# 77even/Fast-nnUNet

Measured on AMD Instinct MI355X. Metric: 3d_fullres patches/sec (distilled r=2 student, sliding window, one 512^3 CT; volume resident in HBM at step start; step ends with: fp16 logits resident in HBM), higher is better.
Workload: dtype f16; 1 GPU; bone_turbo_r2: PlainConvUNet student r=2, features [16, 32, 64, 128, 160, 160], 1 input channel, patch 160x96x96, 61 classes, 512^3 volume, tile_step_size 0.5, Gaussian on, mirroring off, 600 patches/volume; patches_per_forward=32, folds=1, accumulators=fp16, step_output=fp16 logits [heads, X, Y, Z] in HBM (predict_sliding_window_return_logits), gpu_max_hw_queues=4, parallelism=single GPU

## Files before the change

fast-nnunet_amd/csrc/conv3d_row.hip:

```cpp
#include "fnn_device.h"
#include "conv_common.h"
#include <cstdlib>

namespace {

struct RowCur { int n, d, h0, g; };

template <int NBLK, int CH, bool TCONV>
__global__ __launch_bounds__(256, CH == 1 ? (NBLK <= 8 ? 3 : 2) : (NBLK <= 8 ? 2 : 1)) void conv_row_kernel(const ThinParams tp, const int total_units,
                                                                         const int strips, const int SH) {
    extern __shared__ __attribute__((aligned(16))) char smem[];
    const ConvParams &p = tp.c;
    constexpr int W = 16 * NBLK, PB = (W + 2) * 32, RINGB = 12 * PB;
    constexpr int PF = NBLK / 2;
    constexpr int NPL = TCONV ? 1 : CH;
    constexpr int TB = TCONV ? (NBLK + 3) / 4 : 1;
    const int tid = threadIdx.x, lane = tid & 63, r = lane & 15, q = lane >> 4, hl = lane >> 5, kh = q & 1;
    const int wave = __builtin_amdgcn_readfirstlane(tid >> 6);
    const int H = p.Hi, D = p.Di, G = SH >> 2;
    double *sRed = (double *)(smem + CH * RINGB);

    int u_begin, u_end;
    {
        const int nwg = gridDim.x, bid = blockIdx.x;
        const int g = fnn_xcd_tile(nwg, bid);
        u_begin = (int)((long long)total_units * g / nwg);
        u_end = (int)((long long)total_units * (g + 1) / nwg);
    }
    if (u_begin >= u_end) return;
    const int n_groups = (u_end - u_begin) * (G + 1);
    auto advance = [&](RowCur &c) {
        if (++c.g > G) {
            c.g = 0; c.h0 += SH;
            if (c.h0 >= H) { c.h0 = 0; if (++c.d >= D) { c.d = 0; ++c.n; } }
        }
    };

    if (tid < CH * 12 * 4) {
        const int row = tid >> 2, which = (tid >> 1) & 1, half = tid & 1;
        *(f16x8 *)(smem + row * PB + (which ? (W + 1) * 32 : 0) + half * 16) = (f16x8){0, 0, 0, 0, 0, 0, 0, 0};
    }
    for (int i = tid; i < 4 * 16 * 2; i += 256) sRed[i] = 0.0;
    const int cg = tid & 1;
    int e_row[PF], e_goff[PF], e_lds[PF];
#pragma unroll
    for (int u = 0; u < PF; ++u) {
        const int e = tid + 256 * u, i = e / (2 * W), c = e - i * (2 * W), col = (c >> 1) + 1;
        e_row[u] = __builtin_amdgcn_readfirstlane(i);
        e_goff[u] = c * 16;
        e_lds[u] = col * 32 + ((cg ^ ((col >> 2) & 1)) * 16);
    }
    int lanec[5];
#pragma unroll
    for (int ks = 0; ks < 5; ++ks) {
        const int t = 2 * ks + hl < 9 ? 2 * ks + hl : 8;
        const int col = r + t % 3;
        lanec[ks] = col * 32 + ((kh ^ ((col >> 2) & 1)) * 16);
    }
    f16x8 wf[CH][5];
#pragma unroll
    for (int ch = 0; ch < CH; ++ch)
#pragma unroll
        for (int ks = 0; ks < 5; ++ks) wf[ch][ks] = *(const f16x8 *)(p.wpk + ((size_t)(ch * 5 + ks) * 64 + lane) * 8);
    const float4 bv = *(const float4 *)(p.bias + q * 4);
    f16x8 fwf[TCONV ? 4 : 1];
    f32x4 fb = {0.f, 0.f, 0.f, 0.f};
    int up_lds[2] = {0, 0};
    if (TCONV) {
#pragma unroll
        for (int cls = 0; cls < 4; ++cls) fwf[cls] = *(const f16x8 *)(tp.fw + ((size_t)cls * 64 + lane) * 8);
        const float4 t = *(const float4 *)(tp.fbias + q * 4);
        fb = (f32x4){t.x, t.y, t.z, t.w};
#pragma unroll
        for (int jw = 0; jw < 2; ++jw) {
            const int col = 2 * r + jw + 1;
            up_lds[jw] = col * 32 + (((q >> 1) ^ ((col >> 2) & 1)) * 16) + (q & 1) * 8;
        }
    }
    const size_t plane_rows = (size_t)H;
    const int Hl = tp.Hl, Wl = tp.Wl;

    f16x8 xr[NPL][PF];
    f16x8 xl[TB];
    f16x8 sc_h[NPL], sh_h[NPL];
    f16 slope_h[NPL];
    float lsc[8], lsh[8];
#ifndef FNN_NORM_FP32
    f16x8 lsc_h = {0, 0, 0, 0, 0, 0, 0, 0}, lsh_h = lsc_h;
#endif
    int n_ss = -1;
    auto load_ss = [&](int n) {
#pragma unroll
        for (int pc = 0; pc < NPL; ++pc) {
            const SrcDesc &S = p.src[TCONV ? 1 : pc];
            const float *qs, *qh;
            fnn_ss_rows(S.ss, 16, n, 0, p.ident_ss, qs, qh);
#pragma unroll
            for (int j = 0; j < 8; ++j) {
                sc_h[pc][j] = (f16)(cg ? qs[8 + j] : qs[j]);
                sh_h[pc][j] = (f16)(cg ? qh[8 + j] : qh[j]);
            }
            slope_h[pc] = (f16)S.slope;
        }
        if (TCONV) {
            const SrcDesc &S = tp.low;
            const float *qs, *qh;
            fnn_ss_rows(S.ss, 32, n, 0, p.ident_ss, qs, qh);
#pragma unroll
            for (int j = 0; j < 8; ++j) {
                lsc[j] = q == 0 ? qs[j] : q == 1 ? qs[8 + j] : q == 2 ? qs[16 + j] : qs[24 + j];
                lsh[j] = q == 0 ? qh[j] : q == 1 ? qh[8 + j] : q == 2 ? qh[16 + j] : qh[24 + j];
            }
#ifndef FNN_NORM_FP32
#pragma unroll
            for (int j = 0; j < 8; ++j) { lsc_h[j] = (f16)lsc[j]; lsh_h[j] = (f16)lsh[j]; }
#endif
        }
    };
    auto issue = [&](const RowCur &c) {
        const int rbase = c.h0 - 1 + 4 * c.g;
#pragma unroll
        for (int pc = 0; pc < NPL; ++pc) {
            const SrcDesc &S = p.src[TCONV ? 1 : pc];
#pragma unroll
            for (int u = 0; u < PF; ++u) {
                int row = rbase + e_row[u];
                row = row < 0 ? 0 : (row >= H ? H - 1 : row);
                const char *base = (const char *)(S.ptr + (((size_t)c.n * D + c.d) * plane_rows + row) * (W * 16));
                xr[pc][u] = *(const f16x8 *)(base + (unsigned)e_goff[u]);
            }
        }
        if (TCONV) {
            const int lbase = (c.h0 >> 1) - 1 + 2 * c.g;
#pragma unroll
            for (int t = 0; t < TB; ++t) {
                int bb = wave + 4 * t;
                bb = bb < NBLK ? bb : wave;
                const int lr = bb / (NBLK / 2), bl = bb - lr * (NBLK / 2);
                int lrow = lbase + lr;
                lrow = lrow < 0 ? 0 : (lrow >= Hl ? Hl - 1 : lrow);
                const char *base = (const char *)(tp.low.ptr + (size_t)c.n * tp.Dl * Hl * Wl * 32 + (q >> 1) * FNN_CS(tp.low) +
                                                  (((size_t)c.d * Hl + lrow) * Wl) * FNN_VS(tp.low));
                xl[t] = *(const f16x8 *)(base + (unsigned)((16 * bl + r) * (FNN_VS(tp.low) * 2) + (q & 1) * 16));
            }
        }
    };
    auto commit = [&](const RowCur &c, int slot) {
        if (c.n != n_ss) { load_ss(c.n); n_ss = c.n; }
        const int rbase = c.h0 - 1 + 4 * c.g;
#pragma unroll
        for (int pc = 0; pc < NPL; ++pc) {
            char *ring = smem + (TCONV ? 1 : pc) * RINGB;
#pragma unroll
            for (int u = 0; u < PF; ++u) {
                const int row = rbase + e_row[u];
                f16x8 o = xr[pc][u] * sc_h[pc] + sh_h[pc];
                o = __builtin_elementwise_max(o, o * slope_h[pc]);
                if (row < 0 || row >= H) o = (f16x8){0, 0, 0, 0, 0, 0, 0, 0};
                *(f16x8 *)(ring + (slot * 4 + e_row[u]) * PB + e_lds[u]) = o;
            }
        }
        if (TCONV) {
            const int lbase = (c.h0 >> 1) - 1 + 2 * c.g;
            const f16 lslope = (f16)tp.low.slope;
#pragma unroll
            for (int t = 0; t < TB; ++t) {
                const int bb = wave + 4 * t;
                if (bb < NBLK) {
                    const int lr = bb / (NBLK / 2), bl = bb - lr * (NBLK / 2);
                    const int lrow = lbase + lr;
                    const bool ok = lrow >= 0 && lrow < Hl;
#ifdef FNN_NORM_FP32
                    f16x8 o = fnn_norm8(xl[t], lsc, lsh);
#else
                    f16x8 o = xl[t] * lsc_h + lsh_h;
#endif
                    o = __builtin_elementwise_max(o, o * lslope);
                    char *dst = smem + (slot * 4 + 2 * lr) * PB + bl * 1024;
                    f32x4 dd[4];
#pragma unroll
                    for (int cls = 0; cls < 4; ++cls)
                        dd[cls] = __builtin_amdgcn_mfma_f32_16x16x32_f16(fwf[cls], o, (f32x4){0.f, 0.f, 0.f, 0.f}, 0, 0, 0);
                    __builtin_amdgcn_sched_barrier(0);
#pragma unroll
                    for (int cls = 0; cls < 4; ++cls) {
                        f16x4 h;
                        h[0] = (f16)(dd[cls][0] + fb[0]); h[1] = (f16)(dd[cls][1] + fb[1]); h[2] = (f16)(dd[cls][2] + fb[2]); h[3] = (f16)(dd[cls][3] + fb[3]);
                        if (!ok) h = (f16x4){0, 0, 0, 0};
                        *(f16x4 *)(dst + (cls >> 1) * PB + up_lds[cls & 1]) = h;
                    }
                }
            }
        }
    };

    double dsum[4][2];
#pragma unroll
    for (int j = 0; j < 4; ++j) { dsum[j][0] = 0.0; dsum[j][1] = 0.0; }
    auto flush_stats = [&](int n) {
        if (!p.stats_out) return;
#pragma unroll
        for (int j = 0; j < 4; ++j) {
            const double a = row16_sum_f64(dsum[j][0]), b = row16_sum_f64(dsum[j][1]);
            if (r == 0) { double *slot = sRed + (wave * 16 + q * 4 + j) * 2; slot[0] = a; slot[1] = b; }
            dsum[j][0] = 0.0; dsum[j][1] = 0.0;
        }
        __syncthreads();
        if (tid < 32) {
            const int c = tid >> 1, which = tid & 1;
            double v = 0;
#pragma unroll
            for (int w = 0; w < 4; ++w) { v += sRed[(w * 16 + c) * 2 + which]; sRed[(w * 16 + c) * 2 + which] = 0.0; }
            unsafeAtomicAdd(p.stats_out + (((size_t)n * FNN_STAT_REPL + (blockIdx.x & (FNN_STAT_REPL - 1))) * p.Cout + c) * 2 + which, v);
        }
        __syncthreads();
    };

    const unsigned out_lane = (unsigned)((r + 16 * (q & 1)) * 32 + (q >> 1) * 16);
    const f16x2 ones = {(f16)1.f, (f16)1.f};
    auto step = [&](const RowCur &c, int slot) {
        const int slot1 = slot == 2 ? 0 : slot + 1;
        f32x4 acc[NBLK];
#pragma unroll
        for (int b = 0; b < NBLK; ++b) acc[b] = (f32x4){0.f, 0.f, 0.f, 0.f};
#pragma unroll
        for (int ch = 0; ch < CH; ++ch) {
            const int sh0 = (TCONV && ch == 0) ? 1 : 0;
            int ro[3];
#pragma unroll
            for (int tr = 0; tr < 3; ++tr) {
                const int wi = wave + tr + sh0;
                ro[tr] = (wi < 4 ? slot * 4 + wi : slot1 * 4 + wi - 4) * PB;
            }
            const char *ring = smem + ch * RINGB;
#pragma unroll
            for (int ks = 0; ks < 5; ++ks) {
                const int vo = lanec[ks] + (ks == 1 ? (hl ? ro[1] : ro[0]) : ro[ks == 0 ? 0 : ks == 2 ? 1 : 2]);
                constexpr int BG = NBLK <= 8 ? NBLK : NBLK / 2;
#pragma unroll
                for (int b0 = 0; b0 < NBLK; b0 += BG) {
                    f16x8 xf[BG];
#pragma unroll
                    for (int b = 0; b < BG; ++b) xf[b] = *(const f16x8 *)(ring + vo + (b0 + b) * 512);
#pragma unroll
                    for (int b = 0; b < BG; ++b) acc[b0 + b] = __builtin_amdgcn_mfma_f32_16x16x32_f16(wf[ch][ks], xf[b], acc[b0 + b], 0, 0, 0);
                }
            }
        }
        const int orow = c.h0 + 4 * c.g + wave;
        char *obase = (char *)(p.out + (((size_t)c.n * D + c.d) * plane_rows + orow) * (W * 16));
        float t1[4] = {0.f, 0.f, 0.f, 0.f}, t2[4] = {0.f, 0.f, 0.f, 0.f};
#pragma unroll
        for (int b = 0; b < NBLK; b += 2) {
            f16x4 o[2];
#pragma unroll
            for (int h = 0; h < 2; ++h) {
                o[h][0] = (f16)(acc[b + h][0] + bv.x);
                o[h][1] = (f16)(acc[b + h][1] + bv.y);
                o[h][2] = (f16)(acc[b + h][2] + bv.z);
                o[h][3] = (f16)(acc[b + h][3] + bv.w);
            }
            *(fnn_u32x4r *)(obase + out_lane + b * 512) = pair_to_b128(o[0], o[1]);
#pragma unroll
            for (int j = 0; j < 4; ++j) {
                const f16x2 pr = {o[0][j], o[1][j]};
                t1[j] = __builtin_amdgcn_fdot2(pr, ones, t1[j], false);
                t2[j] = __builtin_amdgcn_fdot2(pr, pr, t2[j], false);
            }
        }
        if (p.stats_out) {
#pragma unroll
            for (int j = 0; j < 4; ++j) { dsum[j][0] += (double)t1[j]; dsum[j][1] += (double)t2[j]; }
        }
    };

    RowCur cc;
    {
        const int u = u_begin, strip = u % strips, pd = u / strips;
        cc.h0 = strip * SH; cc.d = pd % D; cc.n = pd / D; cc.g = 0;
    }
    RowCur cw = cc, ci = cc;
    int gw = 0, gl = 0;
    __syncthreads();
    issue(ci);
    commit(cw, 0);
    if (gl < n_groups - 1) { advance(ci); ++gl; }
    if (gw < n_groups - 1) { advance(cw); ++gw; }
    issue(ci);
    commit(cw, 1);
    if (gl < n_groups - 1) { advance(ci); ++gl; }
    if (gw < n_groups - 1) { advance(cw); ++gw; }
    issue(ci);
    __syncthreads();
    int slot = 0;
    for (int gi = 0; gi < n_groups; ++gi) {
        if (cc.g < G) step(cc, slot);
        commit(cw, slot == 0 ? 2 : slot - 1);
        if (gl < n_groups - 1) { advance(ci); ++gl; }
        if (gw < n_groups - 1) { advance(cw); ++gw; }
        issue(ci);
        __syncthreads();
        const int n_prev = cc.n;
        advance(cc);
        slot = slot == 2 ? 0 : slot + 1;
        if (cc.n != n_prev || gi + 1 == n_groups) flush_stats(n_prev);
    }
}

template <int NBLK, bool STORE>
__global__ __launch_bounds__(256, NBLK <= 8 ? 8 : 6) void stem_row_kernel(const StemParams p, const int total_units, const int strips,
                                                           const int SH, const int slots) {
    extern __shared__ __attribute__((aligned(16))) char smem[];
    constexpr int W = 16 * NBLK, PB = W * 8, RINGB = 12 * PB;
    constexpr int PF = (4 * W + 255) / 256;
    const int tid = threadIdx.x, lane = tid & 63, r = lane & 15, q = lane >> 4;
    const int wave = __builtin_amdgcn_readfirstlane(tid >> 6);
    const int H = p.PH, D = p.PD, G = SH >> 2;
    float *sRed = (float *)(smem + RINGB);

    int u_begin, u_end;
    {
        const int nwg = gridDim.x, bid = blockIdx.x;
        const int g = fnn_xcd_tile(nwg, bid);
        u_begin = (int)((long long)total_units * g / nwg);
        u_end = (int)((long long)total_units * (g + 1) / nwg);
    }
    if (u_begin >= u_end) return;
    const int n_groups = (u_end - u_begin) * (G + 1);
    auto advance = [&](RowCur &c) {
        if (++c.g > G) {
            c.g = 0; c.h0 += SH;
            if (c.h0 >= H) { c.h0 = 0; if (++c.d >= D) { c.d = 0; ++c.n; } }
        }
    };
    for (int i = tid; i < RINGB / 16; i += 256) ((uint4 *)smem)[i] = make_uint4(0, 0, 0, 0);

    f16x8 wf = {0, 0, 0, 0, 0, 0, 0, 0};
    {
        const int m = lane & 15;
        if (q == 0) {
#pragma unroll
            for (int t = 0; t < 6; ++t) wf[t + t / 3] = (f16)p.w[(size_t)t * p.Cout + m];
        } else if (q == 1) {
#pragma unroll
            for (int t = 6; t < 9; ++t) wf[t - 6] = (f16)p.w[(size_t)t * p.Cout + m];
        }
    }
    const f32x4 bv = *(const f32x4 *)(p.bias + q * 4);
    int e_row[PF], e_col[PF];
#pragma unroll
    for (int u = 0; u < PF; ++u) {
        const int e = tid + 256 * u, i = e / W;
        e_row[u] = i < 4 ? i : -1;
        e_col[u] = e - i * W;
    }
    float xr[PF];
    const float *voln0 = p.vol;
    int n_org = -1, ox = 0, oy = 0, oz = 0;
    auto issue = [&](const RowCur &c) {
        const int rbase = c.h0 - 1 + 4 * c.g;
        if (c.n != n_org) { ox = p.origins[c.n * 3 + 0]; oy = p.origins[c.n * 3 + 1]; oz = p.origins[c.n * 3 + 2]; n_org = c.n; }
        const int dd = p.flip_d ? D - 1 - c.d : c.d;
        const float *plane = voln0 + (size_t)c.n * p.vol_batch_stride + ((size_t)(ox + dd) * p.Y + oy) * p.Z + oz;
        const unsigned Zu = (unsigned)p.Z;
#pragma unroll
        for (int u = 0; u < PF; ++u) {
            int row = rbase + (e_row[u] < 0 ? 0 : e_row[u]);
            row = row < 0 ? 0 : (row >= H ? H - 1 : row);
            const int hh = p.flip_h ? H - 1 - row : row, ww = p.flip_w ? W - 1 - e_col[u] : e_col[u];
            xr[u] = *(const float *)((const char *)plane + ((unsigned)hh * Zu + (unsigned)ww) * 4u);
        }
    };
    auto commit = [&](const RowCur &c, int slot) {
        const int rbase = c.h0 - 1 + 4 * c.g;
#pragma unroll
        for (int u = 0; u < PF; ++u) {
            if (e_row[u] < 0) continue;
            const int row = rbase + e_row[u];
            const f16 v = (row < 0 || row >= H) ? (f16)0.f : (f16)xr[u];
            char *rowp = smem + (slot * 4 + e_row[u]) * PB;
            const int w = e_col[u];
            *(f16 *)(rowp + w * 8 + 2) = v;
            if (w + 1 < W) *(f16 *)(rowp + (w + 1) * 8) = v;
            if (w > 0) *(f16 *)(rowp + (w - 1) * 8 + 4) = v;
        }
    };

    const unsigned out_lane = (unsigned)((r + 16 * (q & 1)) * 32 + (q >> 1) * 16);
    const f16x2 ones = {(f16)1.f, (f16)1.f};
    float t1[4] = {0.f, 0.f, 0.f, 0.f}, t2[4] = {0.f, 0.f, 0.f, 0.f};
    const unsigned item_bytes = (unsigned)D * H * W * 32;
    auto step = [&](const RowCur &c, int slot, bool valid) {
        const int slot1 = slot == 2 ? 0 : slot + 1;
        int ro[3];
#pragma unroll
        for (int tr = 0; tr < 3; ++tr) {
            const int wi = wave + tr;
            ro[tr] = (wi < 4 ? slot * 4 + wi : slot1 * 4 + wi - 4) * PB;
        }
        const int va = r * 8 + (q == 1 ? ro[2] : ro[0]), vb = r * 8 + (q == 1 ? ro[2] : ro[1]);
        const int orow = c.h0 + 4 * c.g + wave;
        const __amdgpu_buffer_rsrc_t rsrc = __builtin_amdgcn_make_buffer_rsrc(p.out ? p.out + (size_t)c.n * (item_bytes >> 1) : p.out, 0,
                                                                               p.out ? item_bytes : 0u, 0x00020000);
        const unsigned vbase = valid ? out_lane + (unsigned)((c.d * H + orow) * (W * 32)) : 0x80000000u;
#pragma unroll
        for (int b = 0; b < NBLK; b += 2) {
            f16x4 o[2];
#pragma unroll
            for (int h = 0; h < 2; ++h) {
                const f16x4 ea = *(const f16x4 *)(smem + va + (b + h) * 128), eb = *(const f16x4 *)(smem + vb + (b + h) * 128);
                const f16x8 xb = {ea[0], ea[1], ea[2], ea[3], eb[0], eb[1], eb[2], eb[3]};
                const f32x4 dd = __builtin_amdgcn_mfma_f32_16x16x32_f16(wf, xb, bv, 0, 0, 0);
                o[h][0] = (f16)dd[0]; o[h][1] = (f16)dd[1]; o[h][2] = (f16)dd[2]; o[h][3] = (f16)dd[3];
            }
            if (STORE) __builtin_amdgcn_raw_buffer_store_b128(pair_to_b128(o[0], o[1]), rsrc, vbase + b * 512, 0, 0);
            if (valid) {
#pragma unroll
                for (int j = 0; j < 4; ++j) {
                    const f16x2 pr = {o[0][j], o[1][j]};
                    t1[j] = __builtin_amdgcn_fdot2(pr, ones, t1[j], false);
                    t2[j] = __builtin_amdgcn_fdot2(pr, pr, t2[j], false);
                }
            }
        }
    };
    auto unit_stats = [&](const RowCur &c) {
        if (p.stats_out) {
#pragma unroll
            for (int j = 0; j < 4; ++j) {
                const float a = row16_sum(t1[j]), b = row16_sum(t2[j]);
                if (r == 0) { sRed[(wave * 16 + q * 4 + j) * 2] = a; sRed[(wave * 16 + q * 4 + j) * 2 + 1] = b; }
            }
            __syncthreads();
            if (tid < 32) {
                const int ch = tid >> 1, which = tid & 1;
                double v = 0;
#pragma unroll
                for (int w = 0; w < 4; ++w) v += (double)sRed[(w * 16 + ch) * 2 + which];
                const int slot_id = c.d * strips + c.h0 / SH;
                p.stats_out[(((size_t)c.n * slots + slot_id) * p.Cout + ch) * 2 + which] = v;
            }
            __syncthreads();
        }
#pragma unroll
        for (int j = 0; j < 4; ++j) { t1[j] = 0.f; t2[j] = 0.f; }
    };

    RowCur cc;
    {
        const int u = u_begin, strip = u % strips, pd = u / strips;
        cc.h0 = strip * SH; cc.d = pd % D; cc.n = pd / D; cc.g = 0;
    }
    RowCur cw = cc, ci = cc;
    int gw = 0, gl = 0;
    __syncthreads();
    issue(ci);
    commit(cw, 0);
    if (gl < n_groups - 1) { advance(ci); ++gl; }
    if (gw < n_groups - 1) { advance(cw); ++gw; }
    issue(ci);
    commit(cw, 1);
    if (gl < n_groups - 1) { advance(ci); ++gl; }
    if (gw < n_groups - 1) { advance(cw); ++gw; }
    issue(ci);
    __syncthreads();
    int slot = 0;
    for (int gi = 0; gi < n_groups; ++gi) {
        step(cc, slot, cc.g < G);
        commit(cw, slot == 0 ? 2 : slot - 1);
        if (gl < n_groups - 1) { advance(ci); ++gl; }
        if (gw < n_groups - 1) { advance(cw); ++gw; }
        issue(ci);
        __syncthreads();
        if (cc.g == G) unit_stats(cc);
        advance(cc);
        slot = slot == 2 ? 0 : slot + 1;
    }
}

template <int NBLK>
__global__ __launch_bounds__(256, NBLK <= 8 ? 3 : 2) void conv_row_stem_kernel(const ThinParams tp, const int total_units,
                                                                                const int strips, const int SH) {
    extern __shared__ __attribute__((aligned(16))) char smem[];
    const ConvParams &p = tp.c;
    constexpr int W = 16 * NBLK, PB = (W + 2) * 32, RINGB = 12 * PB;
    constexpr int XPB = W * 8, XSLOT = 6 * XPB;
    constexpr int PF = (6 * W + 255) / 256;
    const int tid = threadIdx.x, lane = tid & 63, r = lane & 15, q = lane >> 4, hl = lane >> 5, kh = q & 1;
    const int wave = __builtin_amdgcn_readfirstlane(tid >> 6);
    const int H = p.Hi, D = p.Di, G = SH >> 2;
    char *xring = smem + RINGB;
    double *sRed = (double *)(smem + RINGB + 2 * XSLOT);

    int u_begin, u_end;
    {
        const int nwg = gridDim.x, bid = blockIdx.x;
        const int g = fnn_xcd_tile(nwg, bid);
        u_begin = (int)((long long)total_units * g / nwg);
        u_end = (int)((long long)total_units * (g + 1) / nwg);
    }
    if (u_begin >= u_end) return;
    const int n_groups = (u_end - u_begin) * (G + 1);
    auto advance = [&](RowCur &c) {
        if (++c.g > G) {
            c.g = 0; c.h0 += SH;
            if (c.h0 >= H) { c.h0 = 0; if (++c.d >= D) { c.d = 0; ++c.n; } }
        }
    };

    if (tid < 12 * 4) {
        const int row = tid >> 2, which = (tid >> 1) & 1, half = tid & 1;
        *(f16x8 *)(smem + row * PB + (which ? (W + 1) * 32 : 0) + half * 16) = (f16x8){0, 0, 0, 0, 0, 0, 0, 0};
    }
    for (int i = tid; i < 2 * XSLOT / 16; i += 256) ((uint4 *)xring)[i] = make_uint4(0, 0, 0, 0);
    for (int i = tid; i < 4 * 16 * 2; i += 256) sRed[i] = 0.0;
    int lanec[5];
#pragma unroll
    for (int ks = 0; ks < 5; ++ks) {
        const int t = 2 * ks + hl < 9 ? 2 * ks + hl : 8;
        const int col = r + t % 3;
        lanec[ks] = col * 32 + ((kh ^ ((col >> 2) & 1)) * 16);
    }
    f16x8 wf[5];
#pragma unroll
    for (int ks = 0; ks < 5; ++ks) wf[ks] = *(const f16x8 *)(p.wpk + ((size_t)ks * 64 + lane) * 8);
    const float4 bv = *(const float4 *)(p.bias + q * 4);
    f16x8 swf = {0, 0, 0, 0, 0, 0, 0, 0};
    if (q == 0) {
#pragma unroll
        for (int t = 0; t < 6; ++t) swf[t + t / 3] = tp.fw[(size_t)r * 8 + t];
    } else if (q == 1) {
        swf[0] = tp.fw[(size_t)r * 8 + 6]; swf[1] = tp.fw[(size_t)r * 8 + 7]; swf[2] = tp.fw[(size_t)(16 + r) * 8];
    }
    const f32x4 sbv = *(const f32x4 *)(tp.fbias + q * 4);
    const f16 sslope = (f16)tp.fslope;
    const int st_lds = (r + 1) * 32 + (((q >> 1) ^ (((r + 1) >> 2) & 1)) * 16) + (q & 1) * 8;
    int e_row[PF], e_col[PF];
#pragma unroll
    for (int u = 0; u < PF; ++u) {
        const int e = tid + 256 * u, i = e / W;
        e_row[u] = i < 6 ? i : -1;
        e_col[u] = e - i * W;
    }
    float xr[PF];
    int n_org = -1, ox = 0, oy = 0, oz = 0;
    auto issue = [&](const RowCur &c) {
        const int rbase = c.h0 - 2 + 4 * c.g;
        if (c.n != n_org) { ox = tp.origins[c.n * 3 + 0]; oy = tp.origins[c.n * 3 + 1]; oz = tp.origins[c.n * 3 + 2]; n_org = c.n; }
        const int dd = tp.flip_d ? D - 1 - c.d : c.d;
        const float *plane = tp.vol + (size_t)c.n * tp.vol_batch_stride + ((size_t)(ox + dd) * tp.Y + oy) * tp.Z + oz;
        const unsigned Zu = (unsigned)tp.Z;
#pragma unroll
        for (int u = 0; u < PF; ++u) {
            int row = rbase + (e_row[u] < 0 ? 0 : e_row[u]);
            row = row < 0 ? 0 : (row >= H ? H - 1 : row);
            const int hh = tp.flip_h ? H - 1 - row : row, ww = tp.flip_w ? W - 1 - e_col[u] : e_col[u];
            xr[u] = *(const float *)((const char *)plane + ((unsigned)hh * Zu + (unsigned)ww) * 4u);
        }
    };
    auto xcommit = [&](const RowCur &c, int xs) {
        const int rbase = c.h0 - 2 + 4 * c.g;
#pragma unroll
        for (int u = 0; u < PF; ++u) {
            if (e_row[u] < 0) continue;
            const int row = rbase + e_row[u];
            const f16 v = (row < 0 || row >= H) ? (f16)0.f : (f16)xr[u];
            char *rowp = xring + xs * XSLOT + e_row[u] * XPB;
            const int w = e_col[u];
            *(f16 *)(rowp + w * 8 + 2) = v;
            if (w + 1 < W) *(f16 *)(rowp + (w + 1) * 8) = v;
            if (w > 0) *(f16 *)(rowp + (w - 1) * 8 + 4) = v;
        }
    };
    f16x4 ssc = {0, 0, 0, 0}, ssh = {0, 0, 0, 0};
    int n_ss = -1;
    auto stem_rows = [&](const RowCur &c, int slot, int xs) {
        if (c.n != n_ss) {
            const float *qs = tp.fss + (size_t)(2 * c.n) * 16 + q * 4;
#pragma unroll
            for (int j = 0; j < 4; ++j) { ssc[j] = (f16)qs[j]; ssh[j] = (f16)qs[16 + j]; }
            n_ss = c.n;
        }
        const int row = c.h0 - 1 + 4 * c.g + wave;
        const bool ok = row >= 0 && row < H;
        const char *xb0 = xring + xs * XSLOT + wave * XPB + r * 8;
        const char *pa = xb0 + (q == 1 ? 2 * XPB : 0), *pb = xb0 + (q == 1 ? 2 * XPB : XPB);
        char *dst = smem + (slot * 4 + wave) * PB + st_lds;
        if (!ok) {
#pragma unroll
            for (int b = 0; b < NBLK; ++b) *(f16x4 *)(dst + b * 512) = (f16x4){0, 0, 0, 0};
            return;
        }
        f32x4 dd[NBLK];
#pragma unroll
        for (int b = 0; b < NBLK; ++b) {
            const f16x4 ea = *(const f16x4 *)(pa + b * 128), eb = *(const f16x4 *)(pb + b * 128);
            const f16x8 xb = {ea[0], ea[1], ea[2], ea[3], eb[0], eb[1], eb[2], eb[3]};
            dd[b] = __builtin_amdgcn_mfma_f32_16x16x32_f16(swf, xb, sbv, 0, 0, 0);
        }
        __builtin_amdgcn_sched_barrier(0);
#pragma unroll
        for (int b = 0; b < NBLK; ++b) {
            f16x4 o = {(f16)dd[b][0], (f16)dd[b][1], (f16)dd[b][2], (f16)dd[b][3]};
            o = o * ssc + ssh;
            o = __builtin_elementwise_max(o, o * sslope);
            *(f16x4 *)(dst + b * 512) = o;
        }
    };

    double dsum[4][2];
#pragma unroll
    for (int j = 0; j < 4; ++j) { dsum[j][0] = 0.0; dsum[j][1] = 0.0; }
    auto flush_stats = [&](int n) {
        if (!p.stats_out) return;
#pragma unroll
        for (int j = 0; j < 4; ++j) {
            const double a = row16_sum_f64(dsum[j][0]), b = row16_sum_f64(dsum[j][1]);
            if (r == 0) { double *slot = sRed + (wave * 16 + q * 4 + j) * 2; slot[0] = a; slot[1] = b; }
            dsum[j][0] = 0.0; dsum[j][1] = 0.0;
        }
        __syncthreads();
        if (tid < 32) {
            const int c = tid >> 1, which = tid & 1;
            double v = 0;
#pragma unroll
            for (int w = 0; w < 4; ++w) { v += sRed[(w * 16 + c) * 2 + which]; sRed[(w * 16 + c) * 2 + which] = 0.0; }
            unsafeAtomicAdd(p.stats_out + (((size_t)n * FNN_STAT_REPL + (blockIdx.x & (FNN_STAT_REPL - 1))) * p.Cout + c) * 2 + which, v);
        }
        __syncthreads();
    };
    const unsigned out_lane = (unsigned)((r + 16 * (q & 1)) * 32 + (q >> 1) * 16);
    const f16x2 ones = {(f16)1.f, (f16)1.f};
    const unsigned item_bytes = (unsigned)D * H * W * 32;
    auto step = [&](const RowCur &c, int slot, const bool valid) {
        const int slot1 = slot == 2 ? 0 : slot + 1;
        f16x4 o[NBLK];
#pragma unroll
        for (int b = 0; b < NBLK; ++b) o[b] = (f16x4){0, 0, 0, 0};
      if (valid) {
        f32x4 acc[NBLK];
#pragma unroll
        for (int b = 0; b < NBLK; ++b) acc[b] = (f32x4){0.f, 0.f, 0.f, 0.f};
        int ro[3];
#pragma unroll
        for (int tr = 0; tr < 3; ++tr) {
            const int wi = wave + tr;
            ro[tr] = (wi < 4 ? slot * 4 + wi : slot1 * 4 + wi - 4) * PB;
        }
#pragma unroll
        for (int ks = 0; ks < 5; ++ks) {
            const int vo = lanec[ks] + (ks == 1 ? (hl ? ro[1] : ro[0]) : ro[ks == 0 ? 0 : ks == 2 ? 1 : 2]);
            constexpr int BG = NBLK <= 8 ? NBLK : NBLK / 2;
#pragma unroll
            for (int b0 = 0; b0 < NBLK; b0 += BG) {
                f16x8 xf[BG];
#pragma unroll
                for (int b = 0; b < BG; ++b) xf[b] = *(const f16x8 *)(smem + vo + (b0 + b) * 512);
#pragma unroll
                for (int b = 0; b < BG; ++b) acc[b0 + b] = __builtin_amdgcn_mfma_f32_16x16x32_f16(wf[ks], xf[b], acc[b0 + b], 0, 0, 0);
            }
        }
        float t1[4] = {0.f, 0.f, 0.f, 0.f}, t2[4] = {0.f, 0.f, 0.f, 0.f};
#pragma unroll
        for (int b = 0; b < NBLK; b += 2) {
#pragma unroll
            for (int h = 0; h < 2; ++h) {
                o[b + h][0] = (f16)(acc[b + h][0] + bv.x);
                o[b + h][1] = (f16)(acc[b + h][1] + bv.y);
                o[b + h][2] = (f16)(acc[b + h][2] + bv.z);
                o[b + h][3] = (f16)(acc[b + h][3] + bv.w);
            }
#pragma unroll
            for (int j = 0; j < 4; ++j) {
                const f16x2 pr = {o[b][j], o[b + 1][j]};
                t1[j] = __builtin_amdgcn_fdot2(pr, ones, t1[j], false);
                t2[j] = __builtin_amdgcn_fdot2(pr, pr, t2[j], false);
            }
        }
        if (p.stats_out) {
#pragma unroll
            for (int j = 0; j < 4; ++j) { dsum[j][0] += (double)t1[j]; dsum[j][1] += (double)t2[j]; }
        }
      }
        const int orow = c.h0 + 4 * c.g + wave;
        const __amdgpu_buffer_rsrc_t rsrc = __builtin_amdgcn_make_buffer_rsrc(p.out + (size_t)c.n * (item_bytes >> 1), 0, item_bytes, 0x00020000);
        const unsigned vbase = valid ? out_lane + (unsigned)((c.d * H + orow) * (W * 32)) : 0x80000000u;
        if (valid)
#pragma unroll
        for (int b = 0; b < NBLK; b += 2) __builtin_amdgcn_raw_buffer_store_b128(pair_to_b128(o[b], o[b + 1]), rsrc, vbase + b * 512, 0, 0);
    };

    RowCur cc;
    {
        const int u = u_begin, strip = u % strips, pd = u / strips;
        cc.h0 = strip * SH; cc.d = pd % D; cc.n = pd / D; cc.g = 0;
    }
    RowCur cs = cc, cx = cc, ci = cc;
    int gs = 0, gx = 0, gl = 0;
    auto next = [&](RowCur &c, int &g) { if (g < n_groups - 1) { advance(c); ++g; } };
    __syncthreads();
    issue(ci);
    xcommit(cx, 0); next(cx, gx); next(ci, gl);
    issue(ci);
    __syncthreads();
    stem_rows(cs, 0, 0); next(cs, gs);
    xcommit(cx, 1); next(cx, gx); next(ci, gl);
    issue(ci);
    __syncthreads();
    stem_rows(cs, 1, 1); next(cs, gs);
    xcommit(cx, 0); next(cx, gx); next(ci, gl);
    issue(ci);
    __syncthreads();
    int slot = 0;
    for (int gi = 0; gi < n_groups; ++gi) {
        step(cc, slot, cc.g < G);
        stem_rows(cs, slot == 0 ? 2 : slot - 1, gi & 1); next(cs, gs);
        xcommit(cx, (gi + 1) & 1); next(cx, gx); next(ci, gl);
        issue(ci);
        __syncthreads();
        const int n_prev = cc.n;
        advance(cc);
        slot = slot == 2 ? 0 : slot + 1;
        if (cc.n != n_prev || gi + 1 == n_groups) flush_stats(n_prev);
    }
}

int pick_strips(int H, int &SH) {
    for (int k = 1; k <= 8; ++k)
        if (H % k == 0 && (H / k) % 4 == 0 && H / k <= 64) { SH = H / k; return k; }
    SH = H;
    return 1;
}

template <int NBLK, int CH, bool TCONV>
int launch_row_t(ThinParams tp, hipStream_t st) {
    ConvParams &p = tp.c;
    p.ident_ss = conv3d_identity_ss();
    if (!p.ident_ss) return -2;
    int SH;
    const int strips = pick_strips(p.Hi, SH);
    const int total = p.N * p.Di * strips;
    constexpr int PB = (16 * NBLK + 2) * 32;
    const size_t lds = (size_t)CH * 12 * PB + 4 * 16 * 2 * 8;
    int per_cu = (int)((160 * 1024) / lds);
    static const bool row1_three = fnn_knob("FNN_ROW1_WPC3") != nullptr;
    int cap = CH == 1 ? (NBLK <= 8 ? (row1_three ? 3 : 2) : 2) : (NBLK <= 8 ? 2 : 1);
    static const int wpc_knob = fnn_knob("FNN_ROW_WPC") ? atoi(fnn_knob("FNN_ROW_WPC")) : 0;
    if (wpc_knob > 0 && wpc_knob < cap) cap = wpc_knob;
    if (per_cu > cap) per_cu = cap;
    int gx = 256 * per_cu;
    if (gx > total) gx = total;
    return fnn_launch_lds<conv_row_kernel<NBLK, CH, TCONV>>(dim3(gx), dim3(256), lds, st, tp, total, strips, SH);
}

template <int CH, bool TCONV>
int launch_row_n(const ThinParams &tp, hipStream_t st) {
    switch (tp.c.Wi) {
        case 64: return launch_row_t<4, CH, TCONV>(tp, st);
        case 96: return launch_row_t<6, CH, TCONV>(tp, st);
        case 128: return launch_row_t<8, CH, TCONV>(tp, st);
        case 160: return launch_row_t<10, CH, TCONV>(tp, st);
        case 192: return launch_row_t<12, CH, TCONV>(tp, st);
    }
    return -1;
}

template <int NBLK>
int launch_row_stem_t(ThinParams tp, hipStream_t st) {
    ConvParams &p = tp.c;
    int SH;
    const int strips = pick_strips(p.Hi, SH);
    const int total = p.N * p.Di * strips;
    constexpr int W = 16 * NBLK;
    const size_t lds = (size_t)12 * (W + 2) * 32 + (size_t)2 * 6 * W * 8 + 4 * 16 * 2 * 8;
    int per_cu = (int)((160 * 1024) / lds);
    int cap = NBLK <= 8 ? 3 : 2;
    static const int wpc_knob = fnn_knob("FNN_ROW_WPC") ? atoi(fnn_knob("FNN_ROW_WPC")) : 0;
    if (wpc_knob > 0 && wpc_knob < cap) cap = wpc_knob;
    if (per_cu > cap) per_cu = cap;
    int gx = 256 * per_cu;
    if (gx > total) gx = total;
    return fnn_launch_lds<conv_row_stem_kernel<NBLK>>(dim3(gx), dim3(256), lds, st, tp, total, strips, SH);
}

int launch_row_stem(const ThinParams &tp, hipStream_t st) {
    switch (tp.c.Wi) {
        case 64: return launch_row_stem_t<4>(tp, st);
        case 96: return launch_row_stem_t<6>(tp, st);
        case 128: return launch_row_stem_t<8>(tp, st);
        case 160: return launch_row_stem_t<10>(tp, st);
        case 192: return launch_row_stem_t<12>(tp, st);
    }
    return -1;
}

}

bool row_choose(const ThinParams &tp, const ConvOverrides &o, ConvChoice &c) {
    const ConvParams &p = tp.c;
    if (o.no_row || p.Cout != 16 || p.kd != 1 || p.kh != 3 || p.kw != 3 || p.sd != 1 || p.sh != 1 || p.sw != 1 || p.fp8) return false;
    if (p.Di != p.Do || p.Hi != p.Ho || p.Wi != p.Wo) return false;
    if ((p.Wi != 64 && p.Wi != 96 && p.Wi != 128 && p.Wi != 160 && p.Wi != 192) || p.Hi % 4 != 0 || p.Hi < 8) return false;
    if (tp.fuse == FUSE_TCONV) {
        if (p.n_src != 2 || p.chunks != 2 || p.src[1].C != 16 || tp.low.C != 32) return false;
        if (tp.tsd != 1 || tp.tsh != 2 || tp.tsw != 2 || tp.Dl != p.Di || tp.Hl * 2 != p.Hi || tp.Wl * 2 != p.Wi) return false;
    } else if (tp.fuse == FUSE_STEM) {
        if (o.no_stem_row || p.n_src != 1 || p.chunks != 1 || p.src[0].C != 16) return false;
    } else {
        if (tp.fuse != 0 || p.chunks != p.n_src || p.chunks < 1 || p.chunks > 2) return false;
        for (int i = 0; i < p.n_src; ++i) if (p.src[i].C != 16) return false;
    }
    c.packing = FNN_PACK_LINEAR; c.ksteps = 5; c.chunks = p.chunks;
    c.t[0] = p.Wi / 16;
    if (tp.fuse == FUSE_STEM) {
        c.kernel = CK_ROW_STEM;
        snprintf(c.name, sizeof c.name, "conv_row_stem_kernel<%d>", c.t[0]);
    } else {
        c.kernel = CK_ROW; c.t[1] = tp.fuse == FUSE_TCONV ? 2 : p.chunks; c.t[2] = tp.fuse == FUSE_TCONV;
        snprintf(c.name, sizeof c.name, "conv_row_kernel<%d,%d,%d>", c.t[0], c.t[1], c.t[2]);
    }
    return true;
}

int launch_conv_row(const ThinParams &tp, const ConvChoice &c, hipStream_t st) {
    if (c.kernel == CK_ROW_STEM) return launch_row_stem(tp, st);
    if (c.t[2]) return launch_row_n<2, true>(tp, st);
    return c.t[1] == 1 ? launch_row_n<1, false>(tp, st) : launch_row_n<2, false>(tp, st);
}

bool stem_row_ok(const StemParams &p) {
    const bool off = fnn_knob("FNN_NO_ROW") != nullptr || fnn_knob("FNN_NO_STEM_ROW") != nullptr;
    if (off || p.C != 1 || p.kd != 1 || p.kh != 3 || p.kw != 3 || p.Cout != 16) return false;
    if ((p.PW != 64 && p.PW != 96 && p.PW != 128 && p.PW != 160 && p.PW != 192) || p.PH % 4 != 0 || p.PH < 8) return false;
    if (2ull * p.PD * p.PH * p.PW * 16 >= (1ull << 31) || p.Y * p.Z >= (1ll << 30)) return false;
    int SH;
    const int strips = pick_strips(p.PH, SH);
    return p.PD * strips <= stem_mfma_stats_slots(p.PD, p.PH, p.PW);
}

int launch_stem_row(const StemParams &p, int N, hipStream_t st) {
    if (!stem_row_ok(p)) return -1;
    int SH;
    const int strips = pick_strips(p.PH, SH);
    const int total = N * p.PD * strips, slots = stem_mfma_stats_slots(p.PD, p.PH, p.PW);
    const size_t lds = (size_t)12 * p.PW * 8 + 4 * 16 * 2 * 4;
    static const int wpc = fnn_knob("FNN_STEM_WPC") ? atoi(fnn_knob("FNN_STEM_WPC")) : 8;
    int gx = 256 * wpc;
    if (gx > total) gx = total;
#define STEM_ROW_LAUNCH(NB)                                                                                            \
    do {                                                                                                               \
        fnn_note_kernel("stem_row_kernel<%d,%d>", NB, p.out ? 1 : 0);                                                  \
        if (p.out) hipLaunchKernelGGL((stem_row_kernel<NB, true>), dim3(gx), dim3(256), lds, st, p, total, strips, SH, slots);    \
        else hipLaunchKernelGGL((stem_row_kernel<NB, false>), dim3(gx), dim3(256), lds, st, p, total, strips, SH, slots);         \
    } while (0)
    switch (p.PW) {
        case 64: STEM_ROW_LAUNCH(4); break;
        case 96: STEM_ROW_LAUNCH(6); break;
        case 128: STEM_ROW_LAUNCH(8); break;
        case 160: STEM_ROW_LAUNCH(10); break;
        default: STEM_ROW_LAUNCH(12); break;
    }
#undef STEM_ROW_LAUNCH
    return hipGetLastError() == hipSuccess ? 0 : -2;
}
```

Baseline: 3637 patches/s.

## Load stem input rows one-per-wave and build 3-tap entries with DPP lane shifts

Stem input staging now assigns one input row per wave, with each lane loading whole-row columns. The three horizontal taps per column are built with DPP row shifts plus readlane seams, replacing scattered per-element f16 LDS stores. In the fused row-stem kernel, the double-buffered 6-row input ring becomes a triple-buffered 4-row ring with wraparound indexing, so the prologue needs an extra commit. The goal is cheaper global loads and fewer LDS writes in the input path. The trade-offs are more complex ring indexing and a reliance on DPP semantics. The old path stays available behind FNN_STEM_RING6.

```diff
diff --git a/fast-nnunet_amd/csrc/conv3d_row.hip b/fast-nnunet_amd/csrc/conv3d_row.hip
--- a/fast-nnunet_amd/csrc/conv3d_row.hip
+++ b/fast-nnunet_amd/csrc/conv3d_row.hip
@@ -307,12 +307,48 @@
     }
 }
 
-template <int NBLK, bool STORE>
+template <int W>
+__device__ __forceinline__ void raw_row_offsets(unsigned (&loff)[(W + 63) / 64], const int lane, const int flip_w) {
+    constexpr int NV = (W + 63) / 64;
+#pragma unroll
+    for (int k = 0; k < NV; ++k) {
+        const int col = 64 * k + lane < W ? 64 * k + lane : lane;
+        loff[k] = (unsigned)(flip_w ? W - 1 - col : col) * 4u;
+    }
+}
+template <int W>
+__device__ __forceinline__ void raw_row_load(float (&xr)[(W + 63) / 64], const float *plane, const unsigned Zu, int row, const int H,
+                                             const int flip_h, const unsigned (&loff)[(W + 63) / 64]) {
+    row = row < 0 ? 0 : (row >= H ? H - 1 : row);
+    const char *rowp = (const char *)plane + (size_t)((unsigned)(flip_h ? H - 1 - row : row) * Zu) * 4u;
+#pragma unroll
+    for (int k = 0; k < (W + 63) / 64; ++k) xr[k] = *(const float *)(rowp + loff[k]);
+}
+template <int W>
+__device__ __forceinline__ void raw_row_entries(char *dst, const float (&xr)[(W + 63) / 64], const bool ok, const int lane) {
+    constexpr int NV = (W + 63) / 64, LAST = W - 64 * (NV - 1);
+    unsigned vb[NV];
+#pragma unroll
+    for (int k = 0; k < NV; ++k) {
+        const bool in = ok && (k < NV - 1 || LAST == 64 || lane < LAST);
+        vb[k] = in ? (unsigned)__builtin_bit_cast(unsigned short, (f16)xr[k]) : 0u;
+    }
+#pragma unroll
+    for (int k = 0; k < NV; ++k) {
+        const unsigned seam_l = k > 0 ? (unsigned)__builtin_amdgcn_readlane((int)vb[k - 1], 63) : 0u;
+        const unsigned seam_r = k + 1 < NV ? (unsigned)__builtin_amdgcn_readfirstlane((int)vb[k + 1]) : 0u;
+        const unsigned xl = (unsigned)__builtin_amdgcn_update_dpp((int)seam_l, (int)vb[k], 0x138, 0xf, 0xf, false);
+        const unsigned xh = (unsigned)__builtin_amdgcn_update_dpp((int)seam_r, (int)vb[k], 0x130, 0xf, 0xf, false);
+        if (k < NV - 1 || LAST == 64 || lane < LAST) *(uint2 *)(dst + k * 512) = make_uint2(xl | (vb[k] << 16), xh);
+    }
+}
+
+template <int NBLK, bool STORE, bool RING6>
 __global__ __launch_bounds__(256, NBLK <= 8 ? 8 : 6) void stem_row_kernel(const StemParams p, const int total_units, const int strips,
                                                            const int SH, const int slots) {
     extern __shared__ __attribute__((aligned(16))) char smem[];
     constexpr int W = 16 * NBLK, PB = W * 8, RINGB = 12 * PB;
-    constexpr int PF = (4 * W + 255) / 256;
+    constexpr int PF = RING6 ? (4 * W + 255) / 256 : (W + 63) / 64;
     const int tid = threadIdx.x, lane = tid & 63, r = lane & 15, q = lane >> 4;
     const int wave = __builtin_amdgcn_readfirstlane(tid >> 6);
     const int H = p.PH, D = p.PD, G = SH >> 2;
@@ -348,19 +384,32 @@
     }
     const f32x4 bv = *(const f32x4 *)(p.bias + q * 4);
     int e_row[PF], e_col[PF];
-#pragma unroll
-    for (int u = 0; u < PF; ++u) {
-        const int e = tid + 256 * u, i = e / W;
-        e_row[u] = i < 4 ? i : -1;
-        e_col[u] = e - i * W;
+    unsigned loff[PF];
+    if constexpr (RING6) {
+#pragma unroll
+        for (int u = 0; u < PF; ++u) {
+            const int e = tid + 256 * u, i = e / W;
+            e_row[u] = i < 4 ? i : -1;
+            e_col[u] = e - i * W;
+        }
+    } else {
+        raw_row_offsets<W>(loff, lane, p.flip_w);
     }
     float xr[PF];
     const float *voln0 = p.vol;
     int n_org = -1, ox = 0, oy = 0, oz = 0;
+    int d_pl = -1;
+    const float *plane_c = nullptr;
     auto issue = [&](const RowCur &c) {
         const int rbase = c.h0 - 1 + 4 * c.g;
-        if (c.n != n_org) { ox = p.origins[c.n * 3 + 0]; oy = p.origins[c.n * 3 + 1]; oz = p.origins[c.n * 3 + 2]; n_org = c.n; }
+        const bool new_item = c.n != n_org;
+        if (new_item) { ox = p.origins[c.n * 3 + 0]; oy = p.origins[c.n * 3 + 1]; oz = p.origins[c.n * 3 + 2]; n_org = c.n; }
         const int dd = p.flip_d ? D - 1 - c.d : c.d;
+        if constexpr (!RING6) {
+            if (new_item || c.d != d_pl) { plane_c = voln0 + (size_t)c.n * p.vol_batch_stride + ((size_t)(ox + dd) * p.Y + oy) * p.Z + oz; d_pl = c.d; }
+            raw_row_load<W>(xr, plane_c, (unsigned)p.Z, rbase + wave, H, p.flip_h, loff);
+            return;
+        }
         const float *plane = voln0 + (size_t)c.n * p.vol_batch_stride + ((size_t)(ox + dd) * p.Y + oy) * p.Z + oz;
         const unsigned Zu = (unsigned)p.Z;
 #pragma unroll
@@ -373,6 +422,11 @@
     };
     auto commit = [&](const RowCur &c, int slot) {
         const int rbase = c.h0 - 1 + 4 * c.g;
+        if constexpr (!RING6) {
+            const int row = rbase + wave;
+            raw_row_entries<W>(smem + (slot * 4 + wave) * PB + lane * 8, xr, row >= 0 && row < H, lane);
+            return;
+        }
 #pragma unroll
         for (int u = 0; u < PF; ++u) {
             if (e_row[u] < 0) continue;
@@ -478,19 +532,19 @@
     }
 }
 
-template <int NBLK>
+template <int NBLK, bool RING6>
 __global__ __launch_bounds__(256, NBLK <= 8 ? 3 : 2) void conv_row_stem_kernel(const ThinParams tp, const int total_units,
                                                                                 const int strips, const int SH) {
     extern __shared__ __attribute__((aligned(16))) char smem[];
     const ConvParams &p = tp.c;
     constexpr int W = 16 * NBLK, PB = (W + 2) * 32, RINGB = 12 * PB;
-    constexpr int XPB = W * 8, XSLOT = 6 * XPB;
-    constexpr int PF = (6 * W + 255) / 256;
+    constexpr int XPB = W * 8, XSLOT = (RING6 ? 6 : 4) * XPB;
+    constexpr int PF = RING6 ? (6 * W + 255) / 256 : (W + 63) / 64;
     const int tid = threadIdx.x, lane = tid & 63, r = lane & 15, q = lane >> 4, hl = lane >> 5, kh = q & 1;
     const int wave = __builtin_amdgcn_readfirstlane(tid >> 6);
     const int H = p.Hi, D = p.Di, G = SH >> 2;
     char *xring = smem + RINGB;
-    double *sRed = (double *)(smem + RINGB + 2 * XSLOT);
+    double *sRed = (double *)(smem + RINGB + 12 * XPB);
 
     int u_begin, u_end;
     {
@@ -512,7 +566,7 @@
         const int row = tid >> 2, which = (tid >> 1) & 1, half = tid & 1;
         *(f16x8 *)(smem + row * PB + (which ? (W + 1) * 32 : 0) + half * 16) = (f16x8){0, 0, 0, 0, 0, 0, 0, 0};
     }
-    for (int i = tid; i < 2 * XSLOT / 16; i += 256) ((uint4 *)xring)[i] = make_uint4(0, 0, 0, 0);
+    for (int i = tid; i < 12 * XPB / 16; i += 256) ((uint4 *)xring)[i] = make_uint4(0, 0, 0, 0);
     for (int i = tid; i < 4 * 16 * 2; i += 256) sRed[i] = 0.0;
     int lanec[5];
 #pragma unroll
@@ -536,18 +590,31 @@
     const f16 sslope = (f16)tp.fslope;
     const int st_lds = (r + 1) * 32 + (((q >> 1) ^ (((r + 1) >> 2) & 1)) * 16) + (q & 1) * 8;
     int e_row[PF], e_col[PF];
-#pragma unroll
-    for (int u = 0; u < PF; ++u) {
-        const int e = tid + 256 * u, i = e / W;
-        e_row[u] = i < 6 ? i : -1;
-        e_col[u] = e - i * W;
+    unsigned loff[PF];
+    if constexpr (RING6) {
+#pragma unroll
+        for (int u = 0; u < PF; ++u) {
+            const int e = tid + 256 * u, i = e / W;
+            e_row[u] = i < 6 ? i : -1;
+            e_col[u] = e - i * W;
+        }
+    } else {
+        raw_row_offsets<W>(loff, lane, tp.flip_w);
     }
     float xr[PF];
     int n_org = -1, ox = 0, oy = 0, oz = 0;
+    int d_pl = -1;
+    const float *plane_c = nullptr;
     auto issue = [&](const RowCur &c) {
         const int rbase = c.h0 - 2 + 4 * c.g;
-        if (c.n != n_org) { ox = tp.origins[c.n * 3 + 0]; oy = tp.origins[c.n * 3 + 1]; oz = tp.origins[c.n * 3 + 2]; n_org = c.n; }
+        const bool new_item = c.n != n_org;
+        if (new_item) { ox = tp.origins[c.n * 3 + 0]; oy = tp.origins[c.n * 3 + 1]; oz = tp.origins[c.n * 3 + 2]; n_org = c.n; }
         const int dd = tp.flip_d ? D - 1 - c.d : c.d;
+        if constexpr (!RING6) {
+            if (new_item || c.d != d_pl) { plane_c = tp.vol + (size_t)c.n * tp.vol_batch_stride + ((size_t)(ox + dd) * tp.Y + oy) * tp.Z + oz; d_pl = c.d; }
+            raw_row_load<W>(xr, plane_c, (unsigned)tp.Z, rbase + wave, H, tp.flip_h, loff);
+            return;
+        }
         const float *plane = tp.vol + (size_t)c.n * tp.vol_batch_stride + ((size_t)(ox + dd) * tp.Y + oy) * tp.Z + oz;
         const unsigned Zu = (unsigned)tp.Z;
 #pragma unroll
@@ -560,6 +627,11 @@
     };
     auto xcommit = [&](const RowCur &c, int xs) {
         const int rbase = c.h0 - 2 + 4 * c.g;
+        if constexpr (!RING6) {
+            const int row = rbase + wave;
+            raw_row_entries<W>(xring + (xs * 4 + wave) * XPB + lane * 8, xr, row >= 0 && row < H, lane);
+            return;
+        }
 #pragma unroll
         for (int u = 0; u < PF; ++u) {
             if (e_row[u] < 0) continue;
@@ -583,8 +655,14 @@
         }
         const int row = c.h0 - 1 + 4 * c.g + wave;
         const bool ok = row >= 0 && row < H;
-        const char *xb0 = xring + xs * XSLOT + wave * XPB + r * 8;
-        const char *pa = xb0 + (q == 1 ? 2 * XPB : 0), *pb = xb0 + (q == 1 ? 2 * XPB : XPB);
+        int xo[3];
+#pragma unroll
+        for (int tr = 0; tr < 3; ++tr) {
+            const int wi = wave + tr;
+            xo[tr] = RING6 ? xs * XSLOT + wi * XPB : ((wi < 4 ? xs * 4 + wi : (xs == 2 ? 0 : xs + 1) * 4 + wi - 4)) * XPB;
+        }
+        const char *xb0 = xring + r * 8;
+        const char *pa = xb0 + (q == 1 ? xo[2] : xo[0]), *pb = xb0 + (q == 1 ? xo[2] : xo[1]);
         char *dst = smem + (slot * 4 + wave) * PB + st_lds;
         if (!ok) {
 #pragma unroll
@@ -702,9 +780,10 @@
     issue(ci);
     xcommit(cx, 0); next(cx, gx); next(ci, gl);
     issue(ci);
+    if constexpr (!RING6) { xcommit(cx, 1); next(cx, gx); next(ci, gl); issue(ci); }
     __syncthreads();
     stem_rows(cs, 0, 0); next(cs, gs);
-    xcommit(cx, 1); next(cx, gx); next(ci, gl);
+    xcommit(cx, RING6 ? 1 : 2); next(cx, gx); next(ci, gl);
     issue(ci);
     __syncthreads();
     stem_rows(cs, 1, 1); next(cs, gs);
@@ -714,8 +793,9 @@
     int slot = 0;
     for (int gi = 0; gi < n_groups; ++gi) {
         step(cc, slot, cc.g < G);
-        stem_rows(cs, slot == 0 ? 2 : slot - 1, gi & 1); next(cs, gs);
-        xcommit(cx, (gi + 1) & 1); next(cx, gx); next(ci, gl);
+        const int sp = slot == 0 ? 2 : slot - 1;
+        stem_rows(cs, sp, RING6 ? gi & 1 : sp); next(cs, gs);
+        xcommit(cx, RING6 ? (gi + 1) & 1 : (slot == 2 ? 0 : slot + 1)); next(cx, gx); next(ci, gl);
         issue(ci);
         __syncthreads();
         const int n_prev = cc.n;
@@ -772,7 +852,7 @@
     const int strips = pick_strips(p.Hi, SH);
     const int total = p.N * p.Di * strips;
     constexpr int W = 16 * NBLK;
-    const size_t lds = (size_t)12 * (W + 2) * 32 + (size_t)2 * 6 * W * 8 + 4 * 16 * 2 * 8;
+    const size_t lds = (size_t)12 * (W + 2) * 32 + (size_t)12 * W * 8 + 4 * 16 * 2 * 8;
     int per_cu = (int)((160 * 1024) / lds);
     int cap = NBLK <= 8 ? 3 : 2;
     static const int wpc_knob = fnn_knob("FNN_ROW_WPC") ? atoi(fnn_knob("FNN_ROW_WPC")) : 0;
@@ -780,7 +860,8 @@
     if (per_cu > cap) per_cu = cap;
     int gx = 256 * per_cu;
     if (gx > total) gx = total;
-    return fnn_launch_lds<conv_row_stem_kernel<NBLK>>(dim3(gx), dim3(256), lds, st, tp, total, strips, SH);
+    if (fnn_knob("FNN_STEM_RING6")) return fnn_launch_lds<conv_row_stem_kernel<NBLK, true>>(dim3(gx), dim3(256), lds, st, tp, total, strips, SH);
+    return fnn_launch_lds<conv_row_stem_kernel<NBLK, false>>(dim3(gx), dim3(256), lds, st, tp, total, strips, SH);
 }
 
 int launch_row_stem(const ThinParams &tp, hipStream_t st) {
@@ -845,13 +926,16 @@
     const int total = N * p.PD * strips, slots = stem_mfma_stats_slots(p.PD, p.PH, p.PW);
     const size_t lds = (size_t)12 * p.PW * 8 + 4 * 16 * 2 * 4;
     static const int wpc = fnn_knob("FNN_STEM_WPC") ? atoi(fnn_knob("FNN_STEM_WPC")) : 8;
+    const bool ring6 = fnn_knob("FNN_STEM_RING6") != nullptr;
     int gx = 256 * wpc;
     if (gx > total) gx = total;
 #define STEM_ROW_LAUNCH(NB)                                                                                            \
     do {                                                                                                               \
-        fnn_note_kernel("stem_row_kernel<%d,%d>", NB, p.out ? 1 : 0);                                                  \
-        if (p.out) hipLaunchKernelGGL((stem_row_kernel<NB, true>), dim3(gx), dim3(256), lds, st, p, total, strips, SH, slots);    \
-        else hipLaunchKernelGGL((stem_row_kernel<NB, false>), dim3(gx), dim3(256), lds, st, p, total, strips, SH, slots);         \
+        fnn_note_kernel(ring6 ? "stem_row_kernel<%d,%d,ring6>" : "stem_row_kernel<%d,%d>", NB, p.out ? 1 : 0);        \
+        if (p.out && ring6) hipLaunchKernelGGL((stem_row_kernel<NB, true, true>), dim3(gx), dim3(256), lds, st, p, total, strips, SH, slots);    \
+        else if (p.out) hipLaunchKernelGGL((stem_row_kernel<NB, true, false>), dim3(gx), dim3(256), lds, st, p, total, strips, SH, slots);      \
+        else if (ring6) hipLaunchKernelGGL((stem_row_kernel<NB, false, true>), dim3(gx), dim3(256), lds, st, p, total, strips, SH, slots);      \
+        else hipLaunchKernelGGL((stem_row_kernel<NB, false, false>), dim3(gx), dim3(256), lds, st, p, total, strips, SH, slots);                \
     } while (0)
     switch (p.PW) {
         case 64: STEM_ROW_LAUNCH(4); break;
```

Measured after the change: 3656 patches/s, median of 6. No clear change (+0.5%).

## Rebalance transposed-conv upsample work across waves and pack f32-to-f16 conversions

Applied to the files above, without the earlier changes.

In the fused transposed-conv path, each wave now owns a contiguous range of half-blocks instead of round-robin blocks, which spreads the upsample MFMA work evenly when the block count is odd. Out-of-range rows skip the MFMAs entirely, and the compute and store phases are split so all MFMAs issue before any LDS writes. A shared add_round4 helper does bias add and f16 conversion through packed two-wide converts, used in both the upsample and the main epilogue, to cut conversion instructions. The added dd[TB][4] array raises register pressure, and the new per-wave mapping plus the odd-count skip conditions must exactly cover every LDS row.

```diff
diff --git a/fast-nnunet_amd/csrc/conv3d_row.hip b/fast-nnunet_amd/csrc/conv3d_row.hip
--- a/fast-nnunet_amd/csrc/conv3d_row.hip
+++ b/fast-nnunet_amd/csrc/conv3d_row.hip
@@ -5,6 +5,14 @@
 namespace {
 
 struct RowCur { int n, d, h0, g; };
+
+__device__ __forceinline__ f16x4 add_round4(const f32x4 &a, const f32x4 &b) {
+    typedef float f32x2 __attribute__((ext_vector_type(2)));
+    float s0 = a[0] + b[0], s1 = a[1] + b[1], s2 = a[2] + b[2], s3 = a[3] + b[3];
+    asm("" : "+v"(s0), "+v"(s1), "+v"(s2), "+v"(s3));
+    const f16x2 lo = __builtin_convertvector((f32x2){s0, s1}, f16x2), hi = __builtin_convertvector((f32x2){s2, s3}, f16x2);
+    return (f16x4){lo[0], lo[1], hi[0], hi[1]};
+}
 
 template <int NBLK, int CH, bool TCONV>
 __global__ __launch_bounds__(256, CH == 1 ? (NBLK <= 8 ? 3 : 2) : (NBLK <= 8 ? 2 : 1)) void conv_row_kernel(const ThinParams tp, const int total_units,
@@ -14,7 +22,9 @@
     constexpr int W = 16 * NBLK, PB = (W + 2) * 32, RINGB = 12 * PB;
     constexpr int PF = NBLK / 2;
     constexpr int NPL = TCONV ? 1 : CH;
-    constexpr int TB = TCONV ? (NBLK + 3) / 4 : 1;
+    constexpr int UPW = NBLK / 2;
+    constexpr bool UODD = (UPW & 1) != 0;
+    constexpr int TB = TCONV ? (UPW + 1) / 2 : 1;
     const int tid = threadIdx.x, lane = tid & 63, r = lane & 15, q = lane >> 4, hl = lane >> 5, kh = q & 1;
     const int wave = __builtin_amdgcn_readfirstlane(tid >> 6);
     const int H = p.Hi, D = p.Di, G = SH >> 2;
@@ -62,7 +72,7 @@
     for (int ch = 0; ch < CH; ++ch)
 #pragma unroll
         for (int ks = 0; ks < 5; ++ks) wf[ch][ks] = *(const f16x8 *)(p.wpk + ((size_t)(ch * 5 + ks) * 64 + lane) * 8);
-    const float4 bv = *(const float4 *)(p.bias + q * 4);
+    const f32x4 bv = *(const f32x4 *)(p.bias + q * 4);
     f16x8 fwf[TCONV ? 4 : 1];
     f32x4 fb = {0.f, 0.f, 0.f, 0.f};
     int up_lds[2] = {0, 0};
@@ -134,8 +144,7 @@
             const int lbase = (c.h0 >> 1) - 1 + 2 * c.g;
 #pragma unroll
             for (int t = 0; t < TB; ++t) {
-                int bb = wave + 4 * t;
-                bb = bb < NBLK ? bb : wave;
+                const int bb = (wave * UPW >> 1) + t;
                 const int lr = bb / (NBLK / 2), bl = bb - lr * (NBLK / 2);
                 int lrow = lbase + lr;
                 lrow = lrow < 0 ? 0 : (lrow >= Hl ? Hl - 1 : lrow);
@@ -163,31 +172,45 @@
         if (TCONV) {
             const int lbase = (c.h0 >> 1) - 1 + 2 * c.g;
             const f16 lslope = (f16)tp.low.slope;
+            const bool u_odd = UODD && (wave & 1);
+            f32x4 dd[TB][4];
+            bool ok[TB];
 #pragma unroll
             for (int t = 0; t < TB; ++t) {
-                const int bb = wave + 4 * t;
-                if (bb < NBLK) {
-                    const int lr = bb / (NBLK / 2), bl = bb - lr * (NBLK / 2);
-                    const int lrow = lbase + lr;
-                    const bool ok = lrow >= 0 && lrow < Hl;
+                const int bb = (wave * UPW >> 1) + t;
+                const int lrow = lbase + bb / (NBLK / 2);
+                ok[t] = lrow >= 0 && lrow < Hl;
+                if (!ok[t]) continue;
 #ifdef FNN_NORM_FP32
-                    f16x8 o = fnn_norm8(xl[t], lsc, lsh);
+                f16x8 o = fnn_norm8(xl[t], lsc, lsh);
 #else
-                    f16x8 o = xl[t] * lsc_h + lsh_h;
+                f16x8 o = xl[t] * lsc_h + lsh_h;
 #endif
-                    o = __builtin_elementwise_max(o, o * lslope);
-                    char *dst = smem + (slot * 4 + 2 * lr) * PB + bl * 1024;
-                    f32x4 dd[4];
-#pragma unroll
-                    for (int cls = 0; cls < 4; ++cls)
-                        dd[cls] = __builtin_amdgcn_mfma_f32_16x16x32_f16(fwf[cls], o, (f32x4){0.f, 0.f, 0.f, 0.f}, 0, 0, 0);
-                    __builtin_amdgcn_sched_barrier(0);
-#pragma unroll
-                    for (int cls = 0; cls < 4; ++cls) {
-                        f16x4 h;
-                        h[0] = (f16)(dd[cls][0] + fb[0]); h[1] = (f16)(dd[cls][1] + fb[1]); h[2] = (f16)(dd[cls][2] + fb[2]); h[3] = (f16)(dd[cls][3] + fb[3]);
-                        if (!ok) h = (f16x4){0, 0, 0, 0};
-                        *(f16x4 *)(dst + (cls >> 1) * PB + up_lds[cls & 1]) = h;
+                o = __builtin_elementwise_max(o, o * lslope);
+#pragma unroll
+                for (int rp = 0; rp < 2; ++rp) {
+                    if (UODD && ((t == 0 && rp == 0 && u_odd) || (t == TB - 1 && rp == 1 && !u_odd))) continue;
+#pragma unroll
+                    for (int jw = 0; jw < 2; ++jw)
+                        dd[t][2 * rp + jw] = __builtin_amdgcn_mfma_f32_16x16x32_f16(fwf[2 * rp + jw], o, (f32x4){0.f, 0.f, 0.f, 0.f}, 0, 0, 0);
+                }
+            }
+            __builtin_amdgcn_sched_barrier(0);
+#pragma unroll
+            for (int t = 0; t < TB; ++t) {
+                const int bb = (wave * UPW >> 1) + t;
+                const int lr = bb / (NBLK / 2), bl = bb - lr * (NBLK / 2);
+                char *dst = smem + (slot * 4 + 2 * lr) * PB + bl * 1024;
+#pragma unroll
+                for (int rp = 0; rp < 2; ++rp) {
+                    if (UODD && ((t == 0 && rp == 0 && u_odd) || (t == TB - 1 && rp == 1 && !u_odd))) continue;
+                    if (ok[t]) {
+#pragma unroll
+                        for (int jw = 0; jw < 2; ++jw)
+                            *(f16x4 *)(dst + rp * PB + up_lds[jw]) = add_round4(dd[t][2 * rp + jw], fb);
+                    } else {
+#pragma unroll
+                        for (int jw = 0; jw < 2; ++jw) *(f16x4 *)(dst + rp * PB + up_lds[jw]) = (f16x4){0, 0, 0, 0};
                     }
                 }
             }
@@ -254,12 +277,7 @@
         for (int b = 0; b < NBLK; b += 2) {
             f16x4 o[2];
 #pragma unroll
-            for (int h = 0; h < 2; ++h) {
-                o[h][0] = (f16)(acc[b + h][0] + bv.x);
-                o[h][1] = (f16)(acc[b + h][1] + bv.y);
-                o[h][2] = (f16)(acc[b + h][2] + bv.z);
-                o[h][3] = (f16)(acc[b + h][3] + bv.w);
-            }
+            for (int h = 0; h < 2; ++h) o[h] = add_round4(acc[b + h], bv);
             *(fnn_u32x4r *)(obase + out_lane + b * 512) = pair_to_b128(o[0], o[1]);
 #pragma unroll
             for (int j = 0; j < 4; ++j) {
```

Result: no change. 3651 patches/s before, 3672 patches/s after (median of 6 runs) (+0.6%).
